# cyberlife-coder/velesdb

Measured on AMD Instinct MI355X. Metric: qps_at_recall10_1Mx768_k10, higher is better.
Workload: dtype f32; 1 GPU; 1000000x768 f32 cosine, k=10, exact distance sweep + fused GPU top-k (BASELINE configs[1]); 1024 queries/step, 1024 queries per corpus pass (sweep_topk_gemm_bf16_pp<dot, WIDE> over normalised bf16 images of rows and queries (cosine; ping-po; rows=1000000, dim=768, k=10, parallelism=replicas x1 (query stream split, no collective)

## Files before the change

velesdb_amd/csrc/select_stage.hip:

```cpp
#include <algorithm>
#include <array>
#include <cstdio>
#include <cstdlib>
#include <cstring>
#include <string>
#include <vector>

#include "vdb_probe_env.hpp"
#include "vdb_select_stage.hpp"
#include "vdb_wide.hpp"

namespace vdb {

static inline uint32_t opt_max_tile(const vdb_hip_index* ix) { return (uint32_t)opt_value(ix, VDB_OPT_MAX_QUERY_TILE); }
static inline int opt_engine(const vdb_hip_index* ix) { return (int)opt_value(ix, VDB_OPT_SWEEP_ENGINE); }
static inline int opt_selector(const vdb_hip_index* ix) { return (int)opt_value(ix, VDB_OPT_SELECTOR_LEVEL); }
static const bool g_bf16_seed = [] {
  const char* e = probe_env("VELESDB_BF16_SEED");
  return !(e && e[0] == '0');
}();
static const bool g_pool_select = [] {
  const char* e = probe_env("VELESDB_POOL_SELECT");
  return !(e && e[0] == '0');
}();
// ... 805 lines not shown
  if (ev) (void)hipEventRecord(ev->b, st);
  VDB_HIP(hipGetLastError());
  return VDB_OK;
}


static const bool g_wide_small_k = [] {
  const char* e = probe_env("VELESDB_WIDE_SMALL_K");
  return !(e && e[0] == '0');
}();
static const bool g_wide_fuse = [] {
  const char* e = probe_env("VELESDB_WIDE_FUSE");
  return !(e && e[0] == '0');
}();
int select_level_wide(vdb_hip_index* ix, uint32_t nq_left, uint32_t k, bool sq8) {
  if (opt_selector(ix) < 2 || (!sq8 && opt_engine(ix) != 1) || opt_max_tile(ix) < 128) return 0;
  if (ix->metric != VDB_COSINE && ix->metric != VDB_DOT && (sq8 || ix->metric != VDB_EUCLIDEAN)) return 0;
  if (ix->dim % 64 != 0 || ix->dim < 128 || ix->row_stride != ix->dim) return 0;
  if (k == 0 || k > kWideMaxK || ix->n_rows < kGemmBf16MinRows || ix->n_rows >= 0xFFFFFF00ull) return 0;
  if (k <= kGemmBf16MaxK && (opt_selector(ix) < 3 || !g_wide_small_k)) return 0;
  if (!sq8 && ix->metric != VDB_EUCLIDEAN && sweep_mfma_lds_bytes(1, k, ix->dim) > 160 * 1024) return 0;
  if (!sq8 && ix->metric == VDB_EUCLIDEAN && !l2_gather_fits(ix->dim, k)) return 0;
  if (!select_chunk(nq_left, sq8 ? kSelectMinQueriesSq8 : 0)) return 0;
  if (ix->sel_stats && ix->sel_stats[2] != ix->sel_seq_seen) {
    ix->sel_seq_seen = ix->sel_stats[2];
    if (ix->sel_stats[3] == 4u && (uint64_t)ix->sel_stats[0] * 16 > ix->sel_stats[1]) ix->wide_hold = 64;
  }
  if (ix->wide_hold) {
    ix->wide_hold--;
    return 0;
  }
  return 4;
}

int32_t brute_wide_dev(vdb_hip_index* ix, const float* d_q, uint64_t q_stride, uint32_t nqg, uint32_t k, uint64_t* d_ids, float* d_scores,
                       uint32_t* d_n, hipStream_t st, bool sq8) {
  const bool cosn = !sq8 && cosine_normalised(ix);
  const bool l2 = !sq8 && ix->metric == VDB_EUCLIDEAN;
  const int sel_metric = (cosn || l2) ? VDB_DOT : ix->metric;
  int32_t rc = sq8 ? ensure_sq8_select(ix, st) : (l2 ? ensure_l2_select(ix, st) : (cosn ? ensure_cosn(ix, st) : ensure_sel16(ix, st)));
  if (rc != VDB_OK) return rc;
  const uint32_t dim_a = ix->dim + 64, dim_s = ix->dim + 4;
  const uint16_t* img_rows = sq8 ? ix->sq8_img.as<uint16_t>()
                                 : (l2 ? ix->l2_img.as<uint16_t>() : (cosn ? ix->cosn_img.as<uint16_t>() : ix->rows_bf16.as<uint16_t>()));
  const uint64_t img_stride = l2 ? (uint64_t)dim_a : ((cosn || sq8) ? (uint64_t)ix->dim : ix->bf16_stride);
  const DevBuf& rho_buf = sq8 ? ix->sq8_rho : (l2 ? ix->l2_rho : (cosn ? ix->cosn_rho : ix->bf16_rho));
  const float* sel_norms = sq8 ? ix->sq8_nrm.as<float>() : ix->norms.as<float>();
  DevBuf& list_buf = sq8 ? ix->s_part_cnt : ix->s_fb_keys;
  const uint32_t sel_dim = l2 ? dim_a : ix->dim;
  ix->last_select_level = 4;
  ix->last_kernels |= VDB_KERNEL_SELECT_BF16;
  const uint8_t* alive = ix->any_dead ? ix->alive.as<uint8_t>() : nullptr;
  const uint32_t n = (uint32_t)ix->n_rows, dim = ix->dim;
  static const uint32_t g_small_seed_rows = [] {
    const char* e = probe_env("VELESDB_WIDE_SEED_ROWS");
    const long v = e ? atol(e) : 0;
    return v >= 1024 && v <= (long)kWideSeedRows ? (uint32_t)v / 256u * 256u : kSplitSeedRows;
  }();
  const uint32_t R0 = std::min<uint32_t>(k <= kWideSmallSeedMaxK ? g_small_seed_rows : kWideSeedRows, n), ngrp = (R0 + 15) / 16;
  GemmSchedule sch;
  {
    static const std::array<uint32_t, 3> mult = [] {
      std::array<uint32_t, 3> m{1, 4, 16};
      if (const char* e = probe_env("VELESDB_WIDE_STEPS")) {
        unsigned a = 0, b = 0, c = 0;
        const int got = sscanf(e, "%u,%u,%u", &a, &b, &c);
        m = {got >= 1 ? a : 0u, got >= 2 ? b : 0u, got >= 3 ? c : 0u};
      }
      return m;
    }();
    const uint32_t head[3] = {mult[0], mult[1], mult[2]};
    gemm_schedule(nqg, 0, n, ix->n_cus, head, 0, &sch);
  }
  int g_nqt = 3;
  while (g_nqt > 1 && sweep_mfma_lds_bytes(g_nqt, k, dim) > 160 * 1024) g_nqt--;
  const int g_waves = g_nqt >= 2 ? kMfmaWaves2 : kMfmaWaves1;
  const uint32_t g_B = l2 ? 8u : (uint32_t)g_nqt * 16;
  const uint32_t ntiles16 = (n + 15) / 16;
  const int g_blocks = l2 ? blocks_for(ix, 8, (n + 7) / 8)
                          : (int)std::max<int64_t>(1, std::min<int64_t>(((int64_t)ntiles16 + g_waves - 1) / g_waves, (int64_t)ix->n_cus));
  size_t off = 0;
  auto take = [&](size_t bytes) {
    const size_t o = off;
    off = (off + bytes + 15) & ~(size_t)15;
    return o;
  };
  const size_t o_tau = take((size_t)nqg * 8), o_delta = take((size_t)nqg * 4), o_qn = take((size_t)nqg * 4), o_rho = take((size_t)nqg * 4),
               o_cnt = take((size_t)nqg * 4), o_state = take((size_t)nqg * 4), o_flags = take((size_t)nqg * 4 + 16), o_qmap = take((size_t)nqg * 8),
               o_gid = take((size_t)nqg * k * 8), o_gsc = take((size_t)nqg * k * 4), o_gn = take((size_t)nqg * 4), o_nmax = take(16),
               o_extra = take((size_t)nqg * 4);
  hipError_t e;
  if ((e = ix->s_seed.reserve(off, false, st)) != hipSuccess || (e = list_buf.reserve((size_t)nqg * kWideCap * 8, false, st)) != hipSuccess ||
      (e = ix->s_part_keys.reserve((size_t)nqg * ngrp * 8, false, st)) != hipSuccess ||
      (!sq8 && (e = ix->s_part_cnt.reserve((size_t)nqg * g_blocks * k * 8, false, st)) != hipSuccess) ||
      (e = ix->s_misc.reserve(((size_t)nqg + 256) * img_stride * 2 + (l2 ? (size_t)nqg * dim_s * 4 + 16 : 0), false, st)) != hipSuccess)
    return fail(VDB_ERR_OOM, "wide selection scratch");
  unsigned char* sd = ix->s_seed.as<unsigned char>();
  uint16_t* q16 = ix->s_misc.as<uint16_t>();
  float* qnorms = reinterpret_cast<float*>(sd + o_qn);
  float* rho_q = rho_buf.p ? reinterpret_cast<float*>(sd + o_rho) : nullptr;
  uint32_t* flags = reinterpret_cast<uint32_t*>(sd + o_flags);
  uint32_t* qcount = flags + nqg;
  uint32_t* qmap = reinterpret_cast<uint32_t*>(sd + o_qmap);
  uint32_t* qslot = qmap + nqg;
  uint32_t* norm_max = reinterpret_cast<uint32_t*>(sd + o_nmax);
  EventPair* ev = next_events(ix);
  if (ev) (void)hipEventRecord(ev->a, st);
  if (l2) {
    float* qaug = reinterpret_cast<float*>(ix->s_misc.as<unsigned char>() + ((((size_t)nqg + 256) * img_stride * 2 + 15) & ~(size_t)15));
    launch_l2_augment_queries(d_q, q_stride, q16, dim_a, qaug, dim_s, nqg, dim, st);
    if (rho_q) launch_query_round_error(d_q, q_stride, rho_q, nqg, dim, st);
    PrepArgs pq{};
    pq.rows = d_q;
    pq.norms = qnorms;
    pq.row_stride = q_stride;
    pq.n_rows = nqg;
    pq.dim = dim;
    pq.words = ix->words;
    launch_prep_rows(pq, st);
    VDB_HIP(hipMemsetAsync(flags, 0, (size_t)nqg * 4 + 16, st));
  } else if (cosn) launch_seln_prep_queries(d_q, q_stride, q16, img_stride, qnorms, rho_q, flags, nqg + 4, nqg, dim, st);
  else launch_sel16_prep_queries(d_q, q_stride, q16, img_stride, qnorms, rho_q, flags, nqg + 4, nqg, dim, st);
  if (nqg % 256u) VDB_HIP(hipMemsetAsync(q16 + (size_t)nqg * img_stride, 0, (size_t)256 * img_stride * 2, st));
  if (ix->metric == VDB_DOT || l2) launch_max_norm(sel_norms, n, norm_max, st);
  WideArgs wa{};
  wa.keys = list_buf.as<uint64_t>();
  wa.eps_extra = sq8 ? 1.5e-4f : 0.0f;
  wa.cnt = reinterpret_cast<uint32_t*>(sd + o_cnt);
  wa.state = reinterpret_cast<uint32_t*>(sd + o_state);
  wa.tau = reinterpret_cast<uint64_t*>(sd + o_tau);
  wa.delta = reinterpret_cast<float*>(sd + o_delta);
  wa.qnorms = qnorms;
  wa.rho_q = rho_q;
  wa.rho_max_bits = rho_q ? rho_buf.as<uint32_t>() : nullptr;
  wa.norm_max_bits = norm_max;
  wa.extra = l2 ? reinterpret_cast<float*>(sd + o_extra) : nullptr;
  wa.cap = kWideCap;
  wa.k = k;
  wa.dim = dim;
  launch_seed_scores_bf16(sel_metric, img_rows, img_stride, sel_norms, alive, q16, img_stride, qnorms, ix->s_part_keys.as<uint64_t>(), R0,
                          nqg, sel_dim, st);
  if (l2) launch_wide_seed_l2(wa, ix->s_part_keys.as<uint64_t>(), ngrp, dim_a, nqg, st);
  else launch_wide_seed(ix->metric, wa, ix->s_part_keys.as<uint64_t>(), ngrp, nqg, st);
  for (int j = 0; j < sch.n_launch; j++) {
    EventPair* evs = next_sel_events(ix);
    if (evs) (void)hipEventRecord(evs->a, st);
    e = launch_sweep_gemm_bf16_wide(sel_metric, sch.bp[j], img_rows, img_stride, sel_norms, alive, q16, img_stride, wa.tau, wa.keys, wa.cnt,
                                    wa.cap, sel_dim, nqg, st, qnorms);
    if (evs) (void)hipEventRecord(evs->b, st);
    if (e != hipSuccess) return fail(VDB_ERR_HIP, std::string("wide selection launch: ") + hipGetErrorString(e));
    if (j + 1 < sch.n_launch || l2 || sq8 || !g_wide_fuse) launch_wide_reseed(wa, nqg, st);
  }
  WideOutArgs wo{};
  wo.rows = ix->rows.as<float>();
  wo.norms = ix->norms.as<float>();
  wo.queries = d_q;
  wo.ext_ids = ix->ext_ids.as<uint64_t>();
  wo.out_ids = d_ids;
  wo.out_scores = d_scores;
  wo.out_n = d_n;
  wo.flags = flags;
  wo.qcount = qcount;
  wo.qmap = qmap;
  wo.qslot = qslot;
  wo.row_stride = ix->row_stride;
  wo.q_stride = q_stride;
  wo.dim_pad = (dim + 127) / 128 * 128;
  if (sq8) {
    wo.sq8_codes = ix->sq8_codes.as<uint8_t>();
    wo.sq8_min = ix->sq8_min.as<float>();
    wo.sq8_max = ix->sq8_max.as<float>();
    wo.sq8_nsq = ix->sq8_nsq.as<float>();
    wo.sq8_stride = ix->sq8_stride;
    launch_wide_rerank_sq8(ix->metric, wa, wo, nqg, st);
    SelectFinishArgs fq{};
    fq.flags = flags;
    fq.qcount = qcount;
    fq.qslot = qslot;
    fq.out_ids = d_ids;
    fq.out_scores = d_scores;
    fq.out_n = d_n;
    fq.nq = nqg;
    fq.k = k;
    if (ix->sel_stats) {
      fq.stats_host = ix->sel_stats;
      fq.stats_seq = ++ix->sel_seq;
      fq.stats_level = 4u;
    }
    const int32_t rf = sq8_fallback_flagged(ix, d_q, q_stride, nqg, k, qmap, fq, st);
    if (rf != VDB_OK) return rf;
    ix->split_flags_off = o_flags;
    ix->split_flags_n = nqg;
    ix->split_flags_stream = st;
    if (ev) (void)hipEventRecord(ev->b, st);
// ... 97 lines not shown
```

velesdb_amd/csrc/sweep_gemm_bf16.hip:

```cpp
#include <algorithm>

#include "vdb_probe_env.hpp"
#include "vdb_device.hpp"
#include "vdb_kernels.hpp"

namespace vdb {

typedef float f32x4 __attribute__((ext_vector_type(4)));
typedef __bf16 bf16x8 __attribute__((ext_vector_type(8)));
typedef __attribute__((address_space(3))) void* lds_ptr_t;
typedef __attribute__((address_space(3))) uint32_t lds_u32_t;

constexpr int kG16BM = 256, kG16BN = 256, kG16Waves = 8;
constexpr int kG16Cap = 12;
constexpr int kG16Queue = 39;
#ifndef VDB_G16_DUMP_MAX_LANES
#define VDB_G16_DUMP_MAX_LANES 6
#endif
constexpr int kG16DumpMaxLanes = VDB_G16_DUMP_MAX_LANES;
static_assert(kG16Queue == 39, "g16_protocol.inc keeps two hot lanes' 64 accumulators in queue entries 8 .. 39");
static_assert(kG16Queue <= 64 && kG16Queue >= 32, "the finish pass takes one queue entry per lane; one hot lane's 32 elements fit");
constexpr size_t kOffCand = 131072, kOffTauk = kOffCand + (size_t)kG16BN * kG16Cap * 8, kOffCnts = kOffTauk + kG16BN * 8,
                 kOffQn = kOffCnts + kG16BN * 4, kOffVns = kOffQn + kG16BN * 4, kOffFlags = kOffVns + kG16BM * 4,
                 kOffQueue = kOffFlags + 16,
                 kQueueBytes = 368,
                
                 kG16Lds = kOffQueue + kG16Waves * kQueueBytes;
static_assert(kG16Lds <= 160 * 1024, "LDS budget");
static_assert((size_t)(kG16Queue + 1) * 8 + kG16Queue + 4 <= 364 + 4 && (size_t)(kG16Queue + 1) * 8 + kG16Queue <= 364, "queue layout");

struct Bf16GemmArgs {
  const uint16_t* rows;
  const float* norms;
  const uint8_t* alive;
  const uint16_t* queries;
  const uint64_t* tau0;
  uint64_t* part_keys;
  uint64_t row_stride, q_stride;
  uint32_t n_rows, dim, nq, k;
  uint32_t KT, G, nqt, qper;
  uint32_t row_tile0;
  uint32_t list_stride, list_off;
  const float* qnorms;
  uint64_t* blk_tau;
  const float* qnorms_half;
  unsigned long long* dbg;
  uint64_t* wide_keys;
  uint32_t* wide_cnt;
  uint32_t wide_cap;
};

__device__ __forceinline__ uint32_t lane_now() {
  uint32_t l;
  asm volatile("v_mbcnt_lo_u32_b32 %0, -1, 0\n\tv_mbcnt_hi_u32_b32 %0, -1, %0" : "=v"(l));
  return l;
}

__device__ __forceinline__ void mfma_bf16_inplace(f32x4& c, const f32x4& a, const f32x4& b) {
  asm volatile("v_mfma_f32_16x16x32_bf16 %0, %1, %2, %0" : "+v"(c) : "v"(a), "v"(b));
}
__device__ __forceinline__ void mfma_bf16_first(f32x4& c, const f32x4& a, const f32x4& b) {
  asm volatile("v_mfma_f32_16x16x32_bf16 %0, %1, %2, 0" : "=&v"(c) : "v"(a), "v"(b));
}
__device__ __forceinline__ void mfma_drain() { asm volatile("s_nop 15\n\ts_nop 15" ::: "memory"); }

typedef int i32x4 __attribute__((ext_vector_type(4)));
__device__ __forceinline__ void glds_b128(const i32x4& rsrc, uint32_t voff, uint32_t soff, uint32_t lds_addr) {
  asm volatile("s_mov_b32 m0, %3\n\ts_nop 3\n\tbuffer_load_dwordx4 %0, %1, %2 offen lds"
               :
               : "v"(voff), "s"(rsrc), "s"(soff), "s"(lds_addr)
               : "m0");
}
__device__ __forceinline__ i32x4 make_rsrc(const void* base, uint32_t num_records = 0x7FFFFFFFu) {
  const uint64_t b = reinterpret_cast<uint64_t>(base);
  return i32x4{(int)(uint32_t)b, (int)((uint32_t)(b >> 32) & 0xFFFFu), (int)num_records, 0x00020000};
}
__device__ __forceinline__ i32x4 make_rsrc_uniform(const void* base, uint32_t num_records = 0x7FFFFFFFu) {
  const uint64_t b = reinterpret_cast<uint64_t>(base);
  const uint32_t lo = (uint32_t)__builtin_amdgcn_readfirstlane((int)(uint32_t)b);
  const uint32_t hi = (uint32_t)__builtin_amdgcn_readfirstlane((int)(uint32_t)(b >> 32));
  return i32x4{(int)lo, (int)(hi & 0xFFFFu), __builtin_amdgcn_readfirstlane((int)num_records), 0x00020000};
}
__device__ __forceinline__ uint32_t a_tile_records(uint32_t n_rows, uint32_t rt, uint32_t kt, uint64_t row_stride) {
  const uint64_t left = (uint64_t)(n_rows - rt * (uint32_t)kG16BM) * row_stride * 2u - (uint64_t)kt * 128u;
  return (uint32_t)(left < 0x7FFFFFFFull ? left : 0x7FFFFFFFull);
}
__device__ __forceinline__ uint32_t norm_records(uint32_t n_rows, uint32_t rt) {
  return min(n_rows - rt * (uint32_t)kG16BM, (uint32_t)kG16BM) * 4u;
}
__device__ __forceinline__ void wait_glds() { asm volatile("s_waitcnt vmcnt(0)" ::: "memory"); }

template <int METRIC, bool SPLIT>
__global__ __launch_bounds__(512, 2) void sweep_topk_gemm_bf16_glds(Bf16GemmArgs a) {
  constexpr bool HIB = true;
  constexpr bool WIDE = false;
  constexpr int BM = kG16BM, BN = kG16BN, WAVES = kG16Waves, CAP = kG16Cap, QCAP = kG16Queue;
  extern __shared__ __attribute__((aligned(16))) unsigned char smem[];
  uint64_t* cand = reinterpret_cast<uint64_t*>(smem + kOffCand);
  uint64_t* tauk = reinterpret_cast<uint64_t*>(smem + kOffTauk);
  uint32_t* cnts = reinterpret_cast<uint32_t*>(smem + kOffCnts);
  float* qn = reinterpret_cast<float*>(smem + kOffQn);
  float* vns = reinterpret_cast<float*>(smem + kOffVns);
// ... 166 lines not shown
    for (uint32_t kt = 1; kt + 1 < a.KT; kt++) {
      VDB_G16_STEP(kt, false);
      __syncthreads();
    }
    VDB_G16_STEP(a.KT - 1, false);
    const bool more = it < total;
#define VDB_G16_ACC_F(V) (V)
#include "g16_quicktest.inc"
    if constexpr (METRIC == kHamming || METRIC == kJaccard) {
#include "g16_quicktest_bits.inc"
    } else {
#include "g16_quicktest_dense.inc"
    }
#define VDB_G16_ACC_ELEM(X, A) asm volatile("v_mov_b32 %0, %1" : "=v"(X) : "v"(A))
#define VDB_G16_NO_DUMP 1
#include "g16_protocol.inc"
#undef VDB_G16_NO_DUMP
#undef VDB_G16_ACC_ELEM
#undef VDB_G16_ACC_F
  }
#undef VDB_G16_STEP
#undef VDB_G16_ADVANCE
#undef VDB_G16_GLDS
#undef VDB_G16_REQ
#include "g16_writeout.inc"
}

template <bool FP4, bool F16>
__device__ __forceinline__ void mfma_accv(f32x4& c, const f32x4& a, const f32x4& b) {
  if (FP4)
    asm volatile("v_mfma_scale_f32_16x16x128_f8f6f4 %0, %1, %2, %0, %3, %3 op_sel_hi:[0,0,0] cbsz:4 blgp:4" : "+v"(c) : "v"(a), "v"(b), "v"(0x7F7F7F7Fu));
  else if (F16)
    asm volatile("v_mfma_f32_16x16x32_f16 %0, %1, %2, %0" : "+v"(c) : "v"(a), "v"(b));
  else
    asm volatile("v_mfma_f32_16x16x32_bf16 %0, %1, %2, %0" : "+v"(c) : "v"(a), "v"(b));
}
template <bool FP4, bool F16>
__device__ __forceinline__ void mfma_accv_first(f32x4& c, const f32x4& a, const f32x4& b) {
  if (FP4)
    asm volatile("v_mfma_scale_f32_16x16x128_f8f6f4 %0, %1, %2, 0, %3, %3 op_sel_hi:[0,0,0] cbsz:4 blgp:4" : "=&v"(c) : "v"(a), "v"(b), "v"(0x7F7F7F7Fu));
  else if (F16)
    asm volatile("v_mfma_f32_16x16x32_f16 %0, %1, %2, 0" : "=&v"(c) : "v"(a), "v"(b));
  else
    asm volatile("v_mfma_f32_16x16x32_bf16 %0, %1, %2, 0" : "=&v"(c) : "v"(a), "v"(b));
}
template <int OFF>
__device__ __forceinline__ void lds_frag_read(f32x4& dst, uint32_t addr) {
  asm volatile("ds_read_b128 %0, %1 offset:%2" : "=v"(dst) : "v"(addr), "n"(OFF));
}
__device__ __forceinline__ void pp_barrier_reads_done() { asm volatile("s_waitcnt lgkmcnt(0)\n\ts_barrier" ::: "memory"); }
__device__ __forceinline__ void pp_barrier() { asm volatile("s_barrier" ::: "memory"); }
__device__ __forceinline__ void pp_wait_dma6() { asm volatile("s_waitcnt vmcnt(6)" ::: "memory"); }

template <int METRIC, bool FP4, bool WIDE, bool F16>
__device__ __forceinline__ void gemm16_pp_body(Bf16GemmArgs a) {
  static_assert(!F16 || (!FP4 && !WIDE), "the f16 instance is a result-mode instance");
  static_assert(FP4 == (METRIC == kHamming || METRIC == kJaccard), "the four-bit instance serves the bit metrics, the bf16 instance Cosine / DotProduct");
  constexpr bool HIB = METRIC != kHamming;
  constexpr int BM = kG16BM, BN = kG16BN, WAVES = kG16Waves, CAP = kG16Cap, QCAP = kG16Queue;
  extern __shared__ __attribute__((aligned(16))) unsigned char smem[];
  uint64_t* cand = reinterpret_cast<uint64_t*>(smem + kOffCand);
  uint64_t* tauk = reinterpret_cast<uint64_t*>(smem + kOffTauk);
  uint32_t* cnts = reinterpret_cast<uint32_t*>(smem + kOffCnts);
  float* qn = reinterpret_cast<float*>(smem + kOffQn);
  float* vns = reinterpret_cast<float*>(smem + kOffVns);
  volatile lds_u32_t* flags = (volatile lds_u32_t*)(lds_ptr_t)(smem + kOffFlags);

  const int tid = (int)threadIdx.x;
  const int lane = tid & 63;
  const int wib = __builtin_amdgcn_readfirstlane(tid >> 6);
  const int wr = wib >> 2, wq = wib & 3;
  uint64_t* wq_keys = reinterpret_cast<uint64_t*>(smem + kOffQueue + (size_t)wib * kQueueBytes);
  uint8_t* wq_qs = reinterpret_cast<uint8_t*>(wq_keys + QCAP + 1);

  const uint32_t bid = blockIdx.x;
  const uint32_t xcd = bid & 7u, slot_id = bid >> 3;
  const uint32_t qt = slot_id % a.nqt;
  const uint32_t g = (slot_id / a.nqt) * 8u + xcd;
  const uint32_t q0 = qt * a.qper;
  const uint32_t nq_t = min(a.qper, a.nq - q0);
  const uint32_t k = a.k;
  const uint16_t* queries = a.queries + (size_t)q0 * a.q_stride;

  if (tid < BN) {
    cnts[tid] = 0;
    tauk[tid] = ((uint32_t)tid < nq_t && a.tau0) ? a.tau0[q0 + tid] : kKeyInvalid;
    qn[tid] = 0.0f;
  }
  if (tid < 4) flags[tid] = 0u;
  __syncthreads();
  if (a.qnorms) {
    if ((uint32_t)tid < nq_t) qn[tid] = a.qnorms[q0 + tid];
  } else if (a.qnorms_half) {
    if ((uint32_t)tid < nq_t) qn[tid] = a.qnorms_half[q0 + tid];
  } else {
    for (uint32_t b = wib; b < nq_t; b += WAVES) {
      const uint16_t* qp = queries + (size_t)b * a.q_stride;
      float nacc = 0.0f;
      for (uint32_t c = lane; c * 4 < a.dim; c += 64)
#pragma unroll
        for (int e = 0; e < 4; e++) {
          const uint32_t i = c * 4 + e;
          if (i < a.dim) {
            const float x = F16 ? (float)__builtin_bit_cast(_Float16, qp[i]) : __uint_as_float((uint32_t)qp[i] << 16);
            nacc = __builtin_fmaf(x, x, nacc);
          }
        }
      const float n = sqrtf(butterfly_all(nacc));
      if (lane == 0) qn[b] = n;
// ... 19 lines not shown
    a_rd0 = wr * 128 * 128 + rd_off_; \
    b_rd0 = 32768 + wq * 64 * 128 + rd_off_; \
  } while (0)
  VDB_PP_LANE();
  const uint32_t soff_a = 64u * (uint32_t)a.row_stride * 2u, soff_b = 64u * (uint32_t)a.q_stride * 2u;
  const unsigned char* rows_b = reinterpret_cast<const unsigned char*>(a.rows);
  const unsigned char* queries_b = reinterpret_cast<const unsigned char*>(queries);
  const uint32_t lds0 = (uint32_t)(size_t)(lds_ptr_t)smem;
  const uint32_t lds_w = lds0 + (uint32_t)wib * 1024u;
#define VDB_PP_REQ_A(HALF, RT, KT_, BUF) do { \
    const i32x4 ra_ = make_rsrc_uniform(rows_b + ((size_t)(RT) * BM * a.row_stride + (size_t)(KT_) * 64) * 2, a_tile_records(a.n_rows, (RT), (KT_), a.row_stride)); \
    glds_b128(ra_, voff_a, (uint32_t)(2 * (HALF)) * soff_a, lds_w + (uint32_t)(BUF) * 65536u + (uint32_t)(2 * (HALF)) * 8192u); \
    glds_b128(ra_, voff_a, (uint32_t)(2 * (HALF) + 1) * soff_a, lds_w + (uint32_t)(BUF) * 65536u + (uint32_t)(2 * (HALF) + 1) * 8192u); \
  } while (0)
#define VDB_PP_REQ_B(HALF, KT_, BUF) do { \
    const i32x4 rb_ = make_rsrc_uniform(queries_b + (size_t)(KT_) * 128); \
    glds_b128(rb_, voff_b, (uint32_t)(2 * (HALF)) * soff_b, lds_w + (uint32_t)(BUF) * 65536u + 32768u + (uint32_t)(2 * (HALF)) * 8192u); \
    glds_b128(rb_, voff_b, (uint32_t)(2 * (HALF) + 1) * soff_b, lds_w + (uint32_t)(BUF) * 65536u + 32768u + (uint32_t)(2 * (HALF) + 1) * 8192u); \
  } while (0)

#define VDB_PP_READ_A(DST, RF0, BUF) do { \
    const uint32_t ad0_ = lds0 + (uint32_t)(BUF) * 65536u + (uint32_t)(a_rd0 + rd_x), ad1_ = lds0 + (uint32_t)(BUF) * 65536u + (uint32_t)(a_rd0 + (64 ^ rd_x)); \
    lds_frag_read<((RF0) + 0) * 2048>(DST[0][0], ad0_); lds_frag_read<((RF0) + 0) * 2048>(DST[0][1], ad1_); \
    lds_frag_read<((RF0) + 1) * 2048>(DST[1][0], ad0_); lds_frag_read<((RF0) + 1) * 2048>(DST[1][1], ad1_); \
    lds_frag_read<((RF0) + 2) * 2048>(DST[2][0], ad0_); lds_frag_read<((RF0) + 2) * 2048>(DST[2][1], ad1_); \
    lds_frag_read<((RF0) + 3) * 2048>(DST[3][0], ad0_); lds_frag_read<((RF0) + 3) * 2048>(DST[3][1], ad1_); \
  } while (0)
#define VDB_PP_READ_B(BUF) do { \
    const uint32_t bd0_ = lds0 + (uint32_t)(BUF) * 65536u + (uint32_t)(b_rd0 + rd_x), bd1_ = lds0 + (uint32_t)(BUF) * 65536u + (uint32_t)(b_rd0 + (64 ^ rd_x)); \
    lds_frag_read<0 * 2048>(bv[0][0], bd0_); lds_frag_read<0 * 2048>(bv[0][1], bd1_); \
    lds_frag_read<1 * 2048>(bv[1][0], bd0_); lds_frag_read<1 * 2048>(bv[1][1], bd1_); \
    lds_frag_read<2 * 2048>(bv[2][0], bd0_); lds_frag_read<2 * 2048>(bv[2][1], bd1_); \
    lds_frag_read<3 * 2048>(bv[3][0], bd0_); lds_frag_read<3 * 2048>(bv[3][1], bd1_); \
  } while (0)
#define VDB_PP_MFMA(AV, RF0, T0, FIRST) do { \
_Pragma("unroll") \
    for (int m_ = 0; m_ < 2; m_++) \
_Pragma("unroll") \
      for (int rf_ = 0; rf_ < 4; rf_++) \
_Pragma("unroll") \
        for (int t_ = 0; t_ < 2; t_++) { \
          if ((FIRST) && m_ == 0) mfma_accv_first<FP4, F16>(acc[(RF0) + rf_][(T0) + t_], AV[rf_][m_], bv[(T0) + t_][m_]); \
          else mfma_accv<FP4, F16>(acc[(RF0) + rf_][(T0) + t_], AV[rf_][m_], bv[(T0) + t_][m_]); \
        } \
  } while (0)

  f32x4 acc[8][4];
  f32x4 bv[4][2], a0v[4][2], a1v[4][2];

#include "g16_compact.inc"

  uint32_t qcnt = 0;
  uint32_t epoch = 0;

  uint32_t rt1 = rt_first, kt1 = 0, rt2 = rt_first, kt2 = 0, n2 = 0;
#define VDB_PP_NEXT2() do { \
    rt1 = rt2; \
    kt1 = kt2; \
    if (n2 + 1 < total) { \
      n2++; \
      if (++kt2 == a.KT) { \
        kt2 = 0; \
        rt2 += a.G; \
      } \
    } \
  } while (0)
  uint32_t c = 0;
  if (total) {
    VDB_PP_REQ_A(0, rt_first, 0, 0);
    VDB_PP_REQ_A(1, rt_first, 0, 0);
    VDB_PP_REQ_B(0, 0, 0);
    VDB_PP_REQ_B(1, 0, 0);
    VDB_PP_NEXT2();
    VDB_PP_REQ_B(0, kt2, 1);
    VDB_PP_REQ_A(0, rt2, kt2, 1);
    VDB_PP_REQ_A(1, rt2, kt2, 1);
    VDB_PP_NEXT2();
    pp_wait_dma6();
  }
  pp_barrier();
  if (total) VDB_PP_READ_A(a0v, 0, 0);
  if (wr == 1) pp_barrier();
#ifndef VDB_PP_STAMP
#define VDB_PP_STAMP 0
#endif
#ifndef VDB_PP_STAMP_METRIC
#define VDB_PP_STAMP_METRIC kCosine
#endif
#if VDB_PP_STAMP
  const bool st_on = a.dbg != nullptr && blockIdx.x == 8u && (wib == 0 || wib == 4) && METRIC == VDB_PP_STAMP_METRIC;
  uint32_t st_acc[28] = {0, 0, 0, 0, 0, 0, 0, 0, 0, 0, 0, 0, 0, 0, 0, 0, 0, 0, 0, 0, 0, 0, 0, 0, 0, 0, 0, 0};
  uint32_t st_last = 0;
#define VDB_PP_STAMP_AT(SLOT) do { \
    if (st_on) { \
      uint64_t t_; \
      asm volatile("s_memtime %0\n\ts_waitcnt lgkmcnt(0)" : "=s"(t_)::"memory"); \
      st_acc[SLOT] += (uint32_t)t_ - st_last; \
      st_last = (uint32_t)t_; \
    } \
  } while (0)
#define VDB_PP_STAMP_ISSUE(SLOT) do { if (VDB_PP_STAMP >= 2) VDB_PP_STAMP_AT(SLOT); } while (0)
#define VDB_PP_STAMP_COUNT(SLOT) do { if (st_on) st_acc[SLOT] += 1u; } while (0)
#define VDB_PP_STAMP_ADD(SLOT, N) do { if (st_on) st_acc[SLOT] += (uint32_t)(N); } while (0)
#else
#define VDB_PP_STAMP_AT(SLOT) do { } while (0)
#define VDB_PP_STAMP_ISSUE(SLOT) do { } while (0)
// ... 13 lines not shown
    VDB_PP_STAMP_AT(0); \
    VDB_PP_MFMA(a0v, 0, 0, FIRST); \
    VDB_PP_STAMP_AT(1); \
    pp_barrier(); \
    VDB_PP_STAMP_AT(2); \
     \
    VDB_PP_LPART(VDB_PP_READ_A(a1v, 4, buf), VDB_PP_REQ_B(0, kt2, buf)); \
    VDB_PP_STAMP_ISSUE(3); \
    pp_barrier_reads_done(); \
    VDB_PP_STAMP_AT(0); \
    VDB_PP_MFMA(a0v, 0, 2, FIRST); \
    VDB_PP_STAMP_AT(1); \
    pp_barrier(); \
    VDB_PP_STAMP_AT(2); \
     \
    VDB_PP_REQ_A(0, rt2, kt2, buf); \
    VDB_PP_STAMP_ISSUE(7); \
    pp_wait_dma6(); \
    pp_barrier_reads_done(); \
    VDB_PP_STAMP_AT(4); \
    VDB_PP_MFMA(a1v, 4, 2, FIRST); \
    VDB_PP_STAMP_AT(5); \
    pp_barrier(); \
    VDB_PP_STAMP_AT(6); \
     \
     \
    VDB_PP_LPART(if (!(LAST)) VDB_PP_READ_A(a0v, 0, buf ^ 1u), VDB_PP_REQ_A(1, rt2, kt2, buf)); \
    VDB_PP_STAMP_ISSUE(7); \
    pp_wait_dma6(); \
    pp_barrier_reads_done(); \
    VDB_PP_STAMP_AT(4); \
    VDB_PP_MFMA(a1v, 4, 0, FIRST); \
    VDB_PP_STAMP_AT(5); \
    pp_barrier(); \
    VDB_PP_STAMP_AT(6); \
    VDB_PP_NEXT2(); \
    c++; \
  } while (0)

#if VDB_PP_STAMP
  if (st_on) {
    uint64_t t_;
    asm volatile("s_memtime %0\n\ts_waitcnt lgkmcnt(0)" : "=s"(t_)::"memory");
    st_last = (uint32_t)t_;
  }
#endif
  for (uint32_t rt = rt_first; rt < ntiles; rt += a.G) {
    VDB_PP_KTILE(true, false);
    for (uint32_t kt = 1; kt + 1 < a.KT; kt++) VDB_PP_KTILE(false, false);
    VDB_PP_KTILE(false, true);
    const bool more = c < total;
    if (wr == 0) pp_barrier();
    VDB_PP_STAMP_AT(11);
#define VDB_G16_ACC_F(V) (V)
#include "g16_quicktest.inc"
    if constexpr (METRIC == kHamming || METRIC == kJaccard) {
#include "g16_quicktest_bits.inc"
    } else {
#include "g16_quicktest_dense.inc"
    }
    VDB_PP_STAMP_AT(10);
#define VDB_G16_ACC_ELEM(X, A) asm volatile("v_mov_b32 %0, %1" : "=v"(X) : "v"(A))
#include "g16_protocol.inc"
#undef VDB_G16_ACC_ELEM
#undef VDB_G16_ACC_F
    VDB_PP_LANE();
    VDB_PP_READ_A(a0v, 0, c & 1u);
    if (more && wr == 1) pp_barrier();
    VDB_PP_STAMP_AT(8);
  }
#undef VDB_PP_KTILE
#undef VDB_PP_LANE
#undef VDB_PP_NEXT2
#undef VDB_PP_MFMA
#undef VDB_PP_READ_B
#undef VDB_PP_READ_A
#undef VDB_PP_REQ_B
#undef VDB_PP_REQ_A
  asm volatile("s_waitcnt vmcnt(0)" ::: "memory");
#if VDB_PP_STAMP
  if (st_on && lane_now() == 0) {
    st_acc[9] = c;
    unsigned long long* d = a.dbg + (size_t)(wib == 0 ? 0 : 1) * 28;
    for (int i = 0; i < 28; i++) d[i] = st_acc[i];
  }
#endif
#include "g16_writeout.inc"
}
template <int METRIC, bool FP4 = false, bool WIDE = false>
__global__ __launch_bounds__(512, 2) void sweep_topk_gemm_bf16_pp(Bf16GemmArgs a) { gemm16_pp_body<METRIC, FP4, WIDE, false>(a); }
template <int METRIC>
__global__ __launch_bounds__(512, 2) void sweep_topk_gemm_f16_pp(Bf16GemmArgs a) { gemm16_pp_body<METRIC, false, false, true>(a); }

template <bool F16>
__global__ __launch_bounds__(256) void query_norms_bf16_kernel(const uint16_t* q16, uint64_t q_stride, float* out, uint32_t nq, uint32_t dim) {
  const uint32_t lane = threadIdx.x & 63u, b = blockIdx.x * 4u + (threadIdx.x >> 6);
  if (b >= nq) return;
  const uint16_t* qp = q16 + (size_t)b * q_stride;
  float nacc = 0.0f;
  for (uint32_t c = lane; c * 4 < dim; c += 64)
#pragma unroll
    for (int e = 0; e < 4; e++) {
      const uint32_t i = c * 4 + e;
      if (i < dim) {
        const float x = F16 ? (float)__builtin_bit_cast(_Float16, qp[i]) : __uint_as_float((uint32_t)qp[i] << 16);
        nacc = __builtin_fmaf(x, x, nacc);
      }
    }
  const float n = sqrtf(butterfly_all(nacc));
  if (lane == 0) out[b] = n;
}
void launch_query_norms_bf16(const uint16_t* q16, uint64_t q_stride, float* out, uint32_t nq, uint32_t dim, hipStream_t st, bool f16) {
  if (f16) hipLaunchKernelGGL(query_norms_bf16_kernel<true>, dim3((nq + 3) / 4), dim3(256), 0, st, q16, q_stride, out, nq, dim);
  else hipLaunchKernelGGL(query_norms_bf16_kernel<false>, dim3((nq + 3) / 4), dim3(256), 0, st, q16, q_stride, out, nq, dim);
}

template <bool HIB>
__global__ __launch_bounds__(256) void seed_tau_kernel(const uint64_t* ids, const float* scores, const uint32_t* n, uint64_t* tau0,
                                                       uint64_t* list, uint32_t list_stride, uint32_t nq, uint32_t k) {
  const uint32_t q = blockIdx.x * 256 + threadIdx.x;
  if (q >= nq) return;
  const uint32_t c = min(n[q], k);
  uint64_t t = kKeyInvalid;
  if (c >= k && k > 0) t = make_key<HIB>(scores[(size_t)q * k + k - 1], (uint32_t)ids[(size_t)q * k + k - 1]) + 1ull;
  tau0[q] = t;
  if (list)
    for (uint32_t e = 0; e < k; e++)
      list[(size_t)q * list_stride * k + e] = e < c ? make_key<HIB>(scores[(size_t)q * k + e], (uint32_t)ids[(size_t)q * k + e]) : kKeyInvalid;
}
void launch_seed_tau(const uint64_t* ids, const float* scores, const uint32_t* n, uint64_t* tau0, uint64_t* list,
                     uint32_t list_stride, uint32_t nq, uint32_t k, hipStream_t st, bool hib) {
  if (hib) hipLaunchKernelGGL(seed_tau_kernel<true>, dim3((nq + 255) / 256), dim3(256), 0, st, ids, scores, n, tau0, list, list_stride, nq, k);
  else hipLaunchKernelGGL(seed_tau_kernel<false>, dim3((nq + 255) / 256), dim3(256), 0, st, ids, scores, n, tau0, list, list_stride, nq, k);
}

#if VDB_PP_STAMP
static unsigned long long* g_pp_stamp_buf = nullptr;
static unsigned long long* pp_stamp_dbg() {
  static unsigned long long* dbg = [] {
    void* p = nullptr;
    if (hipMalloc(&p, 512) == hipSuccess) (void)hipMemset(p, 0, 512);
    return static_cast<unsigned long long*>(p);
  }();
  g_pp_stamp_buf = dbg;
  return dbg;
// ... 1 lines not shown
}
extern "C" int32_t vdb_hip_debug_pp_stamps(unsigned long long* out ) {
  if (!vdb::g_pp_stamp_buf) return -1;
  if (hipDeviceSynchronize() != hipSuccess) return -2;
  return hipMemcpy(out, vdb::g_pp_stamp_buf, 448, hipMemcpyDeviceToHost) == hipSuccess ? 0 : -3;
}
namespace vdb {
#endif
static_assert(kG16BM == (int)kGemmTileRows && kG16BN == (int)kGemmTileQueries, "the schedule's tile is the kernel's");

static bool pingpong_enabled() {
  static const bool on = [] {
    const char* e = probe_env("VELESDB_BF16_PP");
    return !(e && e[0] == '0');
  }();
  return on;
}
template <int METRIC>
static hipError_t launch_g16_pp(const Bf16GemmArgs& a, int blocks, hipStream_t st) {
  static bool done = false;
  if (!done) {
    hipError_t e = hipFuncSetAttribute(reinterpret_cast<const void*>(&sweep_topk_gemm_bf16_pp<METRIC>),
                                       hipFuncAttributeMaxDynamicSharedMemorySize, 160 * 1024);
    if (e != hipSuccess) return e;
    done = true;
  }
  hipLaunchKernelGGL((sweep_topk_gemm_bf16_pp<METRIC>), dim3(blocks), dim3(512), kG16Lds, st, a);
  return hipGetLastError();
}

template <int METRIC>
static hipError_t launch_g16_pp_f16(const Bf16GemmArgs& a, int blocks, hipStream_t st) {
  static bool done = false;
  if (!done) {
    hipError_t e = hipFuncSetAttribute(reinterpret_cast<const void*>(&sweep_topk_gemm_f16_pp<METRIC>),
                                       hipFuncAttributeMaxDynamicSharedMemorySize, 160 * 1024);
    if (e != hipSuccess) return e;
    done = true;
  }
  hipLaunchKernelGGL((sweep_topk_gemm_f16_pp<METRIC>), dim3(blocks), dim3(512), kG16Lds, st, a);
  return hipGetLastError();
}

template <int METRIC>
static hipError_t launch_g16_wide(const Bf16GemmArgs& a, int blocks, hipStream_t st) {
  static bool done = false;
  if (!done) {
    hipError_t e = hipFuncSetAttribute(reinterpret_cast<const void*>(&sweep_topk_gemm_bf16_pp<METRIC, false, true>),
                                       hipFuncAttributeMaxDynamicSharedMemorySize, 160 * 1024);
    if (e != hipSuccess) return e;
    done = true;
  }
  hipLaunchKernelGGL((sweep_topk_gemm_bf16_pp<METRIC, false, true>), dim3(blocks), dim3(512), kG16Lds, st, a);
  return hipGetLastError();
}

template <int METRIC>
static hipError_t launch_g16_fp4(const Bf16GemmArgs& a, int blocks, hipStream_t st) {
  static bool done = false;
  if (!done) {
    hipError_t e = hipFuncSetAttribute(reinterpret_cast<const void*>(&sweep_topk_gemm_bf16_pp<METRIC, true>),
                                       hipFuncAttributeMaxDynamicSharedMemorySize, 160 * 1024);
    if (e != hipSuccess) return e;
    done = true;
  }
  hipLaunchKernelGGL((sweep_topk_gemm_bf16_pp<METRIC, true>), dim3(blocks), dim3(512), kG16Lds, st, a);
  return hipGetLastError();
}

template <int METRIC, bool SPLIT>
static hipError_t launch_g16(const Bf16GemmArgs& a, int blocks, hipStream_t st) {
  static bool done = false;
  if (!done) {
    hipError_t e = hipFuncSetAttribute(reinterpret_cast<const void*>(&sweep_topk_gemm_bf16_glds<METRIC, SPLIT>),
                                       hipFuncAttributeMaxDynamicSharedMemorySize, 160 * 1024);
    if (e != hipSuccess) return e;
    done = true;
  }
  hipLaunchKernelGGL((sweep_topk_gemm_bf16_glds<METRIC, SPLIT>), dim3(blocks), dim3(512), kG16Lds, st, a);
  return hipGetLastError();
}

hipError_t launch_sweep_gemm_bf16_wide(int metric, const Bf16GemmPlan& p, const uint16_t* rows16, uint64_t row_stride, const float* norms,
                                       const uint8_t* alive, const uint16_t* queries16, uint64_t q_stride, const uint64_t* tau0,
                                       uint64_t* wide_keys, uint32_t* wide_cnt, uint32_t wide_cap, uint32_t dim, uint32_t nq, hipStream_t st,
                                       const float* qnorms) {
  Bf16GemmArgs a{};
  a.rows = rows16;
  a.norms = norms;
  a.alive = alive;
  a.queries = queries16;
  a.tau0 = tau0;
  a.row_stride = row_stride;
  a.q_stride = q_stride;
  a.n_rows = p.row_hi;
  a.row_tile0 = p.row_lo / kG16BM;
  a.dim = dim;
  a.nq = nq;
  a.k = kGemmBf16MaxK;
  a.KT = dim / 64;
  a.G = p.G;
  a.nqt = p.nqt;
  a.qper = p.qper;
  a.qnorms = qnorms;
  a.wide_keys = wide_keys;
  a.wide_cnt = wide_cnt;
  a.wide_cap = wide_cap;
#if VDB_PP_STAMP
  a.dbg = pp_stamp_dbg();
#endif
  return metric == kCosine ? launch_g16_wide<kCosine>(a, p.blocks, st) : launch_g16_wide<kDot>(a, p.blocks, st);
}

hipError_t launch_sweep_gemm_bf16_glds(int metric, const Bf16GemmPlan& p, const uint16_t* rows16, uint64_t row_stride,
                                       const float* norms, const uint8_t* alive, const uint16_t* queries16, uint64_t q_stride,
                                       const uint64_t* tau0, uint64_t* part_keys, uint32_t list_stride, uint32_t list_off,
                                       uint32_t dim, uint32_t nq, uint32_t k, hipStream_t st, bool split, const float* qnorms,
                                       uint64_t* blk_tau, const float* qnorms_half, bool f16) {
  Bf16GemmArgs a{};
  a.rows = rows16;
  a.norms = norms;
  a.alive = alive;
  a.queries = queries16;
  a.tau0 = tau0;
  a.part_keys = part_keys;
  a.row_stride = row_stride;
  a.q_stride = q_stride;
  a.n_rows = p.row_hi;
  a.row_tile0 = p.row_lo / kG16BM;
  a.list_stride = list_stride;
  a.list_off = list_off;
  a.dim = dim;
  a.nq = nq;
  a.k = k;
  a.KT = split ? dim / 32 : dim / 64;
  a.G = p.G;
  a.nqt = p.nqt;
  a.qper = p.qper;
  a.qnorms = qnorms;
  a.blk_tau = blk_tau;
  a.qnorms_half = qnorms_half;
#if VDB_PP_STAMP
  a.dbg = pp_stamp_dbg();
#endif
  if (f16) {
    if (split || (metric != kCosine && metric != kDot)) return hipErrorInvalidValue;
    return metric == kCosine ? launch_g16_pp_f16<kCosine>(a, p.blocks, st) : launch_g16_pp_f16<kDot>(a, p.blocks, st);
  }
  if (metric == kHamming) return launch_g16_fp4<kHamming>(a, p.blocks, st);
  if (metric == kJaccard) return launch_g16_fp4<kJaccard>(a, p.blocks, st);
  if (split)
    return metric == kCosine ? launch_g16<kCosine, true>(a, p.blocks, st) : launch_g16<kDot, true>(a, p.blocks, st);
  if (pingpong_enabled()) return metric == kCosine ? launch_g16_pp<kCosine>(a, p.blocks, st) : launch_g16_pp<kDot>(a, p.blocks, st);
  return metric == kCosine ? launch_g16<kCosine, false>(a, p.blocks, st) : launch_g16<kDot, false>(a, p.blocks, st);
}

}
```

velesdb_amd/csrc/vdb_wide.hpp:

```cpp
#pragma once
#include <hip/hip_runtime.h>
#include <stdint.h>

#include "vdb_gemm_schedule.hpp"

namespace vdb {

constexpr uint32_t kWideMaxK = 128;
constexpr uint32_t kWideCap = 4096;
constexpr uint32_t kWidePoolMax = 1024;
constexpr uint32_t kWideSeedRows = 16384;
constexpr uint32_t kWideSeedGroups = kWideSeedRows / 16;
constexpr uint32_t kWideSmallSeedMaxK = 32;
constexpr uint32_t kWideGivenUp = 1u;

struct WideArgs {
  uint64_t* keys;
  uint32_t* cnt;
  uint32_t* state;
  uint64_t* tau;
  float* delta;
  const float* qnorms;
  const float* rho_q;
  const uint32_t* rho_max_bits;
  const uint32_t* norm_max_bits;
  float* extra;
  uint32_t cap, k, dim;
  float eps_extra;
};
struct WideOutArgs {
  const float* rows;
  const float* norms;
  const float* queries;
  const uint64_t* ext_ids;
  uint64_t* out_ids;
  float* out_scores;
  uint32_t* out_n;
  uint32_t* flags;
  uint32_t* qcount;
  uint32_t* qmap;
  uint32_t* qslot;
  uint64_t row_stride, q_stride;
  uint32_t dim_pad;
  const uint8_t* sq8_codes;
  const float* sq8_min;
  const float* sq8_max;
  const float* sq8_nsq;
  uint64_t sq8_stride;
  unsigned long long* stamps;
};

void launch_wide_seed(int metric, const WideArgs& a, const uint64_t* seed_keys, uint32_t ngrp, uint32_t nq, hipStream_t st);
void launch_wide_reseed(const WideArgs& a, uint32_t nq, hipStream_t st);
void launch_wide_rerank(int metric, const WideArgs& a, const WideOutArgs& o, uint32_t nq, bool fuse_final_reseed, hipStream_t st);
void launch_wide_seed_l2(const WideArgs& a, const uint64_t* seed_keys, uint32_t ngrp, uint32_t dim_a, uint32_t nq, hipStream_t st);
void launch_wide_rerank_l2(const WideArgs& a, const WideOutArgs& o, uint32_t nq, hipStream_t st);
void launch_wide_rerank_sq8(int metric, const WideArgs& a, const WideOutArgs& o, uint32_t nq, hipStream_t st);
hipError_t launch_sweep_gemm_bf16_wide(int metric, const Bf16GemmPlan& p, const uint16_t* rows16, uint64_t row_stride, const float* norms,
                                       const uint8_t* alive, const uint16_t* queries16, uint64_t q_stride, const uint64_t* tau0,
                                       uint64_t* wide_keys, uint32_t* wide_cnt, uint32_t wide_cap, uint32_t dim, uint32_t nq, hipStream_t st,
                                       const float* qnorms);

}
```

Before: 777,600 queries/s.

## Seed wide selection from a GEMM-based group-max sample instead of seed scores

Adds a sample instance of the ping-pong bf16 GEMM kernel that scores a leading block of rows with MFMA and writes one max-score key per 32 or 64-row group per query. This replaces the separate seed-score kernel for dot-product selection, including normalised cosine. The sample covers more rows, so the starting threshold should be tighter and fewer candidates should reach the wide lists. The default schedule head also changes to {5,16,0} when sampling. The cost is an extra full-tile GEMM pass over the sample rows, and the seed threshold now comes from group maxima rather than individual rows.

```diff
diff --git a/velesdb_amd/csrc/g16_sample.inc b/velesdb_amd/csrc/g16_sample.inc
--- /dev/null
+++ b/velesdb_amd/csrc/g16_sample.inc
@@ -0,0 +1,60 @@
+    mfma_drain();
+    {
+      const uint32_t ln_s = lane_now();
+      const uint32_t kk_s = ln_s >> 4;
+      const uint32_t row_s = rt * (uint32_t)BM + (uint32_t)(wr * 128) + 4u * kk_s;
+      const bool pair_s = a.sample_grp == 64u;
+      const uint32_t grp_s = pair_s ? (rt - a.row_tile0) * 4u + (uint32_t)wr * 2u + (kk_s >> 1) : (rt - a.row_tile0) * 8u + (uint32_t)wr * 4u + kk_s;
+      const bool slow_s = a.alive != nullptr || a.n_rows - rt * (uint32_t)BM < (uint32_t)BM;
+      uint32_t live_s = 0xFFFFFFFFu;
+      uint32_t first_s = row_s;
+      if (slow_s) {
+        live_s = 0u;
+#pragma unroll
+        for (int e = 0; e < 32; e++) {
+          const uint32_t row = row_s + (uint32_t)((e >> 2) * 16 + (e & 3));
+          bool lv = row < a.n_rows;
+          if (lv && a.alive) lv = a.alive[row] != 0;
+          live_s |= lv ? 1u << e : 0u;
+        }
+        const uint32_t e0 = live_s ? (uint32_t)__builtin_ctz(live_s) : 0u;
+        first_s = live_s ? row_s + (e0 >> 2) * 16u + (e0 & 3u) : 0xFFFFFFFFu;
+      }
+      if (pair_s) {
+        auto r_ = __builtin_amdgcn_permlane16_swap(first_s, first_s, false, false);
+        first_s = min((uint32_t)r_[0], (uint32_t)r_[1]);
+      }
+#define VDB_SMP_MAX3(M, A, B, C) asm volatile("v_max3_f32 %0, %1, %2, %3" : "=v"(M) : "v"(A), "v"(B), "v"(C))
+#pragma unroll
+      for (int t = 0; t < 4; t++) {
+        float mx;
+        if (!slow_s) {
+          float m_[8];
+#pragma unroll
+          for (int rf = 0; rf < 8; rf++) VDB_SMP_MAX3(m_[rf], acc[rf][t][0], acc[rf][t][1], acc[rf][t][2]);
+#pragma unroll
+          for (int j = 0; j < 4; j++) VDB_SMP_MAX3(m_[j], m_[2 * j], m_[2 * j + 1], acc[2 * j][t][3]);
+          VDB_SMP_MAX3(m_[0], m_[0], m_[1], acc[1][t][3]);
+          VDB_SMP_MAX3(m_[2], m_[2], m_[3], acc[3][t][3]);
+          VDB_SMP_MAX3(m_[0], m_[0], m_[2], acc[5][t][3]);
+          VDB_SMP_MAX3(mx, m_[0], acc[7][t][3], acc[7][t][3]);
+        } else {
+          mx = __uint_as_float(0xFF800000u);
+#pragma unroll
+          for (int e = 0; e < 32; e++) {
+            float x;
+            asm volatile("v_mov_b32 %0, %1" : "=v"(x) : "v"(acc[e >> 2][t][e & 3]));
+            if ((live_s >> e) & 1u) mx = fmaxf(mx, x);
+          }
+        }
+        if (pair_s) {
+          auto r_ = __builtin_amdgcn_permlane16_swap(__float_as_uint(mx), __float_as_uint(mx), false, false);
+          mx = fmaxf(__uint_as_float(r_[0]), __uint_as_float(r_[1]));
+        }
+        const uint64_t key = (mx > __uint_as_float(0xFF800000u) && first_s != 0xFFFFFFFFu) ? make_key<true>(mx, first_s) : kKeyInvalid;
+        const uint32_t b = (uint32_t)(wq * 64 + t * 16) + (ln_s & 15u);
+        if (b < nq_t && grp_s < a.list_stride && !(pair_s && (kk_s & 1u))) a.part_keys[(size_t)(q0 + b) * a.list_stride + grp_s] = key;
+      }
+#undef VDB_SMP_MAX3
+    }
+    __syncthreads();
diff --git a/velesdb_amd/csrc/select_stage.hip b/velesdb_amd/csrc/select_stage.hip
--- a/velesdb_amd/csrc/select_stage.hip
+++ b/velesdb_amd/csrc/select_stage.hip
@@ -881,24 +881,44 @@
   ix->last_kernels |= VDB_KERNEL_SELECT_BF16;
   const uint8_t* alive = ix->any_dead ? ix->alive.as<uint8_t>() : nullptr;
   const uint32_t n = (uint32_t)ix->n_rows, dim = ix->dim;
+  static const bool g_wide_sample = [] {
+    const char* e = probe_env("VELESDB_WIDE_SAMPLE");
+    return !(e && e[0] == '0');
+  }();
+  static const uint32_t g_sample_tiles = [] {
+    const char* e = probe_env("VELESDB_WIDE_SAMPLE_TILES");
+    const long v = e ? atol(e) : 0;
+    return v >= 1 && v <= 4 ? (uint32_t)v : 1u;
+  }();
+  static const uint32_t g_sample_group = [] {
+    const char* e = probe_env("VELESDB_WIDE_SAMPLE_GROUP");
+    const long v = e ? atol(e) : 0;
+    return v == 32 || v == 64 ? (uint32_t)v : kWideSampleGroupRows;
+  }();
+  WideSamplePlan smp{};
+  if (g_wide_sample && sel_metric == VDB_DOT) wide_sample_plan(nqg, n, k, g_sample_tiles, g_sample_group, &smp);
+  const bool sample = smp.rows != 0;
   static const uint32_t g_small_seed_rows = [] {
     const char* e = probe_env("VELESDB_WIDE_SEED_ROWS");
     const long v = e ? atol(e) : 0;
     return v >= 1024 && v <= (long)kWideSeedRows ? (uint32_t)v / 256u * 256u : kSplitSeedRows;
   }();
-  const uint32_t R0 = std::min<uint32_t>(k <= kWideSmallSeedMaxK ? g_small_seed_rows : kWideSeedRows, n), ngrp = (R0 + 15) / 16;
+  const uint32_t R0 = std::min<uint32_t>(k <= kWideSmallSeedMaxK ? g_small_seed_rows : kWideSeedRows, n);
+  const uint32_t ngrp = sample ? smp.ngrp : (R0 + 15) / 16;
   GemmSchedule sch;
   {
-    static const std::array<uint32_t, 3> mult = [] {
-      std::array<uint32_t, 3> m{1, 4, 16};
+    static const std::array<uint32_t, 4> mult = [] {
+      std::array<uint32_t, 4> m{0, 0, 0, 0};
       if (const char* e = probe_env("VELESDB_WIDE_STEPS")) {
         unsigned a = 0, b = 0, c = 0;
         const int got = sscanf(e, "%u,%u,%u", &a, &b, &c);
-        m = {got >= 1 ? a : 0u, got >= 2 ? b : 0u, got >= 3 ? c : 0u};
+        m = {got >= 1 ? a : 0u, got >= 2 ? b : 0u, got >= 3 ? c : 0u, 1u};
       }
       return m;
     }();
-    const uint32_t head[3] = {mult[0], mult[1], mult[2]};
+    const uint32_t head_seed[3] = {1, 4, 16};
+    const uint32_t* dflt = sample ? kWideSampleHead : head_seed;
+    const uint32_t head[3] = {mult[3] ? mult[0] : dflt[0], mult[3] ? mult[1] : dflt[1], mult[3] ? mult[2] : dflt[2]};
     gemm_schedule(nqg, 0, n, ix->n_cus, head, 0, &sch);
   }
   int g_nqt = 3;
@@ -967,8 +987,17 @@
   wa.cap = kWideCap;
   wa.k = k;
   wa.dim = dim;
-  launch_seed_scores_bf16(sel_metric, img_rows, img_stride, sel_norms, alive, q16, img_stride, qnorms, ix->s_part_keys.as<uint64_t>(), R0,
-                          nqg, sel_dim, st);
+  if (sample) {
+    EventPair* evs = next_sel_events(ix);
+    if (evs) (void)hipEventRecord(evs->a, st);
+    e = launch_sweep_gemm_bf16_sample(smp.bp, img_rows, img_stride, sel_norms, alive, q16, img_stride, ix->s_part_keys.as<uint64_t>(), ngrp, smp.grp_rows,
+                                      sel_dim, nqg, st, qnorms);
+    if (evs) (void)hipEventRecord(evs->b, st);
+    if (e != hipSuccess) return fail(VDB_ERR_HIP, std::string("wide sample launch: ") + hipGetErrorString(e));
+  } else {
+    launch_seed_scores_bf16(sel_metric, img_rows, img_stride, sel_norms, alive, q16, img_stride, qnorms, ix->s_part_keys.as<uint64_t>(), R0, nqg,
+                            sel_dim, st);
+  }
   if (l2) launch_wide_seed_l2(wa, ix->s_part_keys.as<uint64_t>(), ngrp, dim_a, nqg, st);
   else launch_wide_seed(ix->metric, wa, ix->s_part_keys.as<uint64_t>(), ngrp, nqg, st);
   for (int j = 0; j < sch.n_launch; j++) {
diff --git a/velesdb_amd/csrc/sweep_gemm_bf16.hip b/velesdb_amd/csrc/sweep_gemm_bf16.hip
--- a/velesdb_amd/csrc/sweep_gemm_bf16.hip
+++ b/velesdb_amd/csrc/sweep_gemm_bf16.hip
@@ -48,6 +48,7 @@
   uint64_t* wide_keys;
   uint32_t* wide_cnt;
   uint32_t wide_cap;
+  uint32_t sample_grp;
 };
 
 __device__ __forceinline__ uint32_t lane_now() {
@@ -320,9 +321,10 @@
 __device__ __forceinline__ void pp_barrier() { asm volatile("s_barrier" ::: "memory"); }
 __device__ __forceinline__ void pp_wait_dma6() { asm volatile("s_waitcnt vmcnt(6)" ::: "memory"); }
 
-template <int METRIC, bool FP4, bool WIDE, bool F16>
+template <int METRIC, bool FP4, bool WIDE, bool F16, bool SAMPLE = false>
 __device__ __forceinline__ void gemm16_pp_body(Bf16GemmArgs a) {
   static_assert(!F16 || (!FP4 && !WIDE), "the f16 instance is a result-mode instance");
+  static_assert(!SAMPLE || (METRIC == kDot && !FP4 && !WIDE && !F16), "the sample instance serves the selections whose metric is DotProduct");
   static_assert(FP4 == (METRIC == kHamming || METRIC == kJaccard), "the four-bit instance serves the bit metrics, the bf16 instance Cosine / DotProduct");
   constexpr bool HIB = METRIC != kHamming;
   constexpr int BM = kG16BM, BN = kG16BN, WAVES = kG16Waves, CAP = kG16Cap, QCAP = kG16Queue;
@@ -448,6 +450,15 @@
 
   uint32_t qcnt = 0;
   uint32_t epoch = 0;
+  if constexpr (SAMPLE) {
+    (void)compact;
+    (void)qcnt;
+    (void)epoch;
+    (void)cand;
+    (void)flags;
+    (void)wq_qs;
+    (void)k;
+  }
 
   uint32_t rt1 = rt_first, kt1 = 0, rt2 = rt_first, kt2 = 0, n2 = 0;
 #define VDB_PP_NEXT2() do { \
@@ -567,6 +578,9 @@
     const bool more = c < total;
     if (wr == 0) pp_barrier();
     VDB_PP_STAMP_AT(11);
+    if constexpr (SAMPLE) {
+#include "g16_sample.inc"
+    } else {
 #define VDB_G16_ACC_F(V) (V)
 #include "g16_quicktest.inc"
     if constexpr (METRIC == kHamming || METRIC == kJaccard) {
@@ -579,6 +593,7 @@
 #include "g16_protocol.inc"
 #undef VDB_G16_ACC_ELEM
 #undef VDB_G16_ACC_F
+    }
     VDB_PP_LANE();
     VDB_PP_READ_A(a0v, 0, c & 1u);
     if (more && wr == 1) pp_barrier();
@@ -600,12 +615,15 @@
     for (int i = 0; i < 28; i++) d[i] = st_acc[i];
   }
 #endif
+  if constexpr (!SAMPLE) {
 #include "g16_writeout.inc"
+  }
 }
 template <int METRIC, bool FP4 = false, bool WIDE = false>
 __global__ __launch_bounds__(512, 2) void sweep_topk_gemm_bf16_pp(Bf16GemmArgs a) { gemm16_pp_body<METRIC, FP4, WIDE, false>(a); }
 template <int METRIC>
 __global__ __launch_bounds__(512, 2) void sweep_topk_gemm_f16_pp(Bf16GemmArgs a) { gemm16_pp_body<METRIC, false, false, true>(a); }
+__global__ __launch_bounds__(512, 2) void sweep_topk_sample_bf16_pp(Bf16GemmArgs a) { gemm16_pp_body<kDot, false, false, false, true>(a); }
 
 template <bool F16>
 __global__ __launch_bounds__(256) void query_norms_bf16_kernel(const uint16_t* q16, uint64_t q_stride, float* out, uint32_t nq, uint32_t dim) {
@@ -713,6 +731,17 @@
     done = true;
   }
   hipLaunchKernelGGL((sweep_topk_gemm_bf16_pp<METRIC, false, true>), dim3(blocks), dim3(512), kG16Lds, st, a);
+  return hipGetLastError();
+}
+
+static hipError_t launch_g16_sample(const Bf16GemmArgs& a, int blocks, hipStream_t st) {
+  static bool done = false;
+  if (!done) {
+    hipError_t e = hipFuncSetAttribute(reinterpret_cast<const void*>(&sweep_topk_sample_bf16_pp), hipFuncAttributeMaxDynamicSharedMemorySize, 160 * 1024);
+    if (e != hipSuccess) return e;
+    done = true;
+  }
+  hipLaunchKernelGGL(sweep_topk_sample_bf16_pp, dim3(blocks), dim3(512), kG16Lds, st, a);
   return hipGetLastError();
 }
 
@@ -771,6 +800,35 @@
   a.dbg = pp_stamp_dbg();
 #endif
   return metric == kCosine ? launch_g16_wide<kCosine>(a, p.blocks, st) : launch_g16_wide<kDot>(a, p.blocks, st);
+}
+
+hipError_t launch_sweep_gemm_bf16_sample(const Bf16GemmPlan& p, const uint16_t* rows16, uint64_t row_stride, const float* norms, const uint8_t* alive,
+                                         const uint16_t* queries16, uint64_t q_stride, uint64_t* keys, uint32_t ngrp, uint32_t grp_rows, uint32_t dim,
+                                         uint32_t nq, hipStream_t st, const float* qnorms) {
+  if ((grp_rows != 32 && grp_rows != 64) || p.row_lo % kG16BM || p.row_hi <= p.row_lo ||
+      (uint64_t)ngrp * grp_rows < ((uint64_t)(p.row_hi - p.row_lo) + kG16BM - 1) / kG16BM * kG16BM)
+    return hipErrorInvalidValue;
+  Bf16GemmArgs a{};
+  a.rows = rows16;
+  a.norms = norms;
+  a.alive = alive;
+  a.queries = queries16;
+  a.part_keys = keys;
+  a.list_stride = ngrp;
+  a.sample_grp = grp_rows;
+  a.row_stride = row_stride;
+  a.q_stride = q_stride;
+  a.n_rows = p.row_hi;
+  a.row_tile0 = p.row_lo / kG16BM;
+  a.dim = dim;
+  a.nq = nq;
+  a.k = kGemmBf16MaxK;
+  a.KT = dim / 64;
+  a.G = p.G;
+  a.nqt = p.nqt;
+  a.qper = p.qper;
+  a.qnorms = qnorms;
+  return launch_g16_sample(a, p.blocks, st);
 }
 
 hipError_t launch_sweep_gemm_bf16_glds(int metric, const Bf16GemmPlan& p, const uint16_t* rows16, uint64_t row_stride,
diff --git a/velesdb_amd/csrc/vdb_wide.hpp b/velesdb_amd/csrc/vdb_wide.hpp
--- a/velesdb_amd/csrc/vdb_wide.hpp
+++ b/velesdb_amd/csrc/vdb_wide.hpp
@@ -3,6 +3,7 @@
 #include <stdint.h>
 
 #include "vdb_gemm_schedule.hpp"
+#include "vdb_wide_sample.hpp"
 
 namespace vdb {
 
@@ -12,6 +13,7 @@
 constexpr uint32_t kWideSeedRows = 16384;
 constexpr uint32_t kWideSeedGroups = kWideSeedRows / 16;
 constexpr uint32_t kWideSmallSeedMaxK = 32;
+static_assert(kWideSampleMaxKeys == kWideSeedGroups && kWideSampleSmallK == kWideSmallSeedMaxK, "vdb_wide_sample.hpp restates them");
 constexpr uint32_t kWideGivenUp = 1u;
 
 struct WideArgs {
@@ -60,5 +62,8 @@
                                        const uint8_t* alive, const uint16_t* queries16, uint64_t q_stride, const uint64_t* tau0,
                                        uint64_t* wide_keys, uint32_t* wide_cnt, uint32_t wide_cap, uint32_t dim, uint32_t nq, hipStream_t st,
                                        const float* qnorms);
+hipError_t launch_sweep_gemm_bf16_sample(const Bf16GemmPlan& p, const uint16_t* rows16, uint64_t row_stride, const float* norms, const uint8_t* alive,
+                                         const uint16_t* queries16, uint64_t q_stride, uint64_t* keys, uint32_t ngrp, uint32_t grp_rows, uint32_t dim,
+                                         uint32_t nq, hipStream_t st, const float* qnorms);
 
 }
diff --git a/velesdb_amd/csrc/vdb_wide_sample.hpp b/velesdb_amd/csrc/vdb_wide_sample.hpp
--- /dev/null
+++ b/velesdb_amd/csrc/vdb_wide_sample.hpp
@@ -0,0 +1,42 @@
+#pragma once
+#include <stdint.h>
+
+#include <algorithm>
+
+#include "vdb_gemm_schedule.hpp"
+
+namespace vdb {
+
+constexpr uint32_t kWideSampleRows = 16384;
+constexpr uint32_t kWideSampleRowsLargeK = 32768;
+constexpr uint32_t kWideSampleSmallK = 32;
+constexpr uint32_t kWideSampleGroupRows = 64;
+constexpr uint32_t kWideSampleMaxKeys = 1024;
+constexpr uint32_t kWideSampleHead[3] = {5, 16, 0};
+
+struct WideSamplePlan {
+  Bf16GemmPlan bp;
+  uint32_t rows;
+  uint32_t grp_rows;
+  uint32_t ngrp;
+};
+
+inline void wide_sample_plan(uint32_t nq, uint32_t n, uint32_t k, uint32_t tiles_per_block, uint32_t grp_rows, WideSamplePlan* s) {
+  tiles_per_block = std::max(1u, tiles_per_block);
+  grp_rows = grp_rows == 32 ? 32u : 64u;
+  uint32_t rows = (k <= kWideSampleSmallK ? kWideSampleRows : kWideSampleRowsLargeK) * tiles_per_block;
+  rows = std::min(rows, kWideSampleMaxKeys * grp_rows);
+  rows = std::min(rows, n / kGemmTileRows * kGemmTileRows);
+  const uint32_t tiles = rows / kGemmTileRows;
+  s->rows = rows;
+  s->grp_rows = grp_rows;
+  s->ngrp = rows / grp_rows;
+  s->bp.nqt = (nq + kGemmTileQueries - 1) / kGemmTileQueries;
+  s->bp.qper = s->bp.nqt ? (nq + s->bp.nqt - 1) / s->bp.nqt : 0;
+  s->bp.row_lo = 0;
+  s->bp.row_hi = rows;
+  s->bp.G = (std::max(1u, tiles / tiles_per_block) + 7) / 8 * 8;
+  s->bp.blocks = (int)(s->bp.G * s->bp.nqt);
+}
+
+}
```

New measurement: 790,100 queries/s, median of 6. +1.6%, better.
